# micahvista/VACmap

Measured on AMD Instinct MI355X. Metric: aligned Gbp/s (whole node) + reads/s, 15 kb ONT-shape reads vs hg38-size ref, 1/2/4/8 MI355X, higher is better.
Workload: dtype i16/i32 DP + f64 chains

## Files before the change

### include/vacmapx.h

```cpp
#ifndef VACMAPX_H
#define VACMAPX_H
#include <stdint.h>
#ifdef __cplusplus
extern "C" {
#endif

typedef enum vm_status {
    VM_OK = 0,
    VM_ERR_ARG = -1,
    VM_ERR_NO_DEVICE = -2,
    VM_ERR_NO_CTX = -3,
    VM_ERR_OOM = -4,
    VM_ERR_IO = -5,
    VM_ERR_HIP = -6,
    VM_ERR_UNSUPPORTED = -7,
    VM_READ_RAISED = -10,
    VM_READ_CAPACITY = -20,
    VM_READ_FASTPATH = -21,
    VM_READ_UNSUPPORTED = -22
} vm_status;

enum { VM_MODE_H = 0, VM_MODE_L = 1, VM_MODE_S = 2, VM_MODE_R = 3,
       VM_MODE_ASM = 4 };

// ... 65 lines not shown
    double* S; int64_t* P; int64_t* S_arg; int64_t* gmax; int64_t* opcount;
} vm_chains_out;
int vm_chain_global_batch(vm_ctx*, const vm_params*, int kmersize, int64_t n, const int64_t* anchors,
                          const int64_t* anchor_off, const int64_t* readlens, int want_raw, vm_chains_out* out);
void vm_chains_out_free(vm_chains_out*);

typedef struct vm_local_out {
    int32_t* status;
    int32_t* variant;
    double* score;
    int64_t* chain_off;
    int64_t* chain;
    int64_t* raw_off;
    int64_t* raw;
} vm_local_out;
int vm_local_chain_batch(vm_ctx*, const vm_index*, const vm_params*, int64_t n, const char* seqs, const int64_t* offsets,
                         const int64_t* read_path_off, const int64_t* path_off, const int64_t* path_anchors, vm_local_out* out);
void vm_local_out_free(vm_local_out*);

typedef struct vm_linked_out {
    int64_t gmax, n_hot, n_cold, opcount; double cold_max;
    double* S; int64_t* P; int64_t* S_arg_hot;
    int32_t carry_status, saved; int64_t n_carry; double* carry_S; int64_t* carry_P; int64_t* carry_rows; double carry_g_max_scores; int64_t carry_prereadloc;
} vm_linked_out;
int vm_chain_linked(vm_ctx*, int which, int kmersize, double skipcost, int maxdiff, int maxgap, int64_t n, const int64_t* rows, int64_t n_pre,
                    const double* pre_S, const int64_t* pre_P, double g_max_scores, int64_t g_max_index, int64_t prereadloc, vm_linked_out* out);
void vm_linked_out_free(vm_linked_out*);

typedef struct vm_score { int32_t match, mismatch, o1, e1, o2, e2; } vm_score;
int vm_k_cigar_batch(vm_ctx*, const vm_score*, int eqx, int64_t n, const char* t, const int64_t* t_off, const char* q,
                     const int64_t* q_off, char** cigars, int64_t** cigar_off, int32_t** scores);
int vm_k_cigar_batch_banded(vm_ctx*, const vm_score*, int eqx, int64_t n, const char* t, const int64_t* t_off, const char* q,
                            const int64_t* q_off, char** cigars, int64_t** cigar_off, int32_t** band_flag, int64_t* stats);
int vm_k_extend_batch(vm_ctx*, int match, int mismatch, int o, int e, int bw, int zdrop, int64_t n, const char* t,
                      const int64_t* t_off, const char* q, const int64_t* q_off, int32_t** t_e, int32_t** q_e, int32_t** score);
typedef struct vm_cigar_out { char* cigar; int32_t q_e, t_e, score; } vm_cigar_out;
int vm_k_cigar(vm_ctx*, const char* t, int64_t tl, const char* q, int64_t ql, const vm_score* sc, int bw, int zdrop,
               int eqx, vm_cigar_out* out);
int vm_edit_distance_batch(vm_ctx*, int64_t n, const char* q, const int64_t* q_off, const char* t, const int64_t* t_off,
                           int64_t** dist);
int64_t vm_edit_distance(vm_ctx*, const char* q, int64_t ql, const char* t, int64_t tl);
int vm_edit_distance_bound_batch(vm_ctx*, int tier, int64_t n, const char* q, const int64_t* q_off, const char* t, const int64_t* t_off,
                                 int64_t** bound);

typedef struct vm_record {
    int32_t read_idx;
    int32_t contig;
    int32_t strand;
    int32_t mapq;
    int64_t q_st, q_en;
    int64_t r_st, r_en;
    int64_t cigar_off, cigar_len;
} vm_record;

typedef struct vm_batch_stats {
    int64_t n_reads, read_bases, n_minimizers, n_hits, n_anchors, n_local_hits, n_local_anchors;
    int64_t n_segments, n_ed_problems, ed_cells, n_ext_problems, ext_cells, n_dp_problems, dp_cells;
    int64_t n_records, cigar_bytes, aligned_bases, n_unmapped, n_failed;
    int64_t dp_string_bytes;
    double ms_total;
    double ms_stage[16];
    double ms_gapfill_fill;
    double ms_gapfill_trace;
    int64_t n_gapfill_launches;
    int64_t n_ed_full;
    int64_t n_ed_tier2;
// ... 76 lines not shown
```

### vacmap_amd/csrc/k_dp.hip

```cpp
#include "vmx_device.h"
#include "vmx_kernels.h"

__device__ __forceinline__ int vmx_tcode(uint8_t c) { return c < 4 ? (int)c : 6; }


__global__ void k_encode(const char* __restrict__ in, uint8_t* __restrict__ out, int64_t n) {
    int64_t i = (int64_t)blockIdx.x * blockDim.x + threadIdx.x;
    int64_t stride = (int64_t)gridDim.x * blockDim.x;
    for (; i < n; i += stride) out[i] = vmx_code((uint8_t)in[i]);
}

#define VMX_EXT_RING 512
__global__ void __launch_bounds__(64) k_extend(const uint8_t* __restrict__ tcodes, const int64_t* __restrict__ t_off,
                                               const uint8_t* __restrict__ qcodes, const int64_t* __restrict__ q_off, int n_prob,
                                               int match, int mismatch, int o, int e, int bw_in, int zdrop,
                                               int32_t* __restrict__ out_te, int32_t* __restrict__ out_qe, int32_t* __restrict__ out_sc, const int32_t* __restrict__ n_ptr) {
    if (n_ptr) n_prob = *n_ptr;
    __shared__ int sH[3][VMX_EXT_RING];
    __shared__ int sE[2][VMX_EXT_RING];
    __shared__ int sF[2][VMX_EXT_RING];
    const int lane = vmx_lane();
    const int RM = VMX_EXT_RING - 1;
    for (int p = blockIdx.x; p < n_prob; p += gridDim.x) {
        const uint8_t* T = tcodes + t_off[p];
// ... 239 lines not shown
                    sHE = (unsigned)vmx_r16_ror1((int)vmx_bfi(l15, (outH >> 16) | (outE1 & 0xffff0000u), sHE));                    \
                    sE2 = (unsigned)vmx_r16_ror1((int)vmx_bfi(l15, outE2 >> 16, sE2));                                             \
                    if ((TT) == 14) {       \
                        const int colr = t + 14 - 30 - l;           \
                        const int col = colr;                                                                                      \
                        if (store_bnd && act && colr >= 1 && col <= ql) { bH[col] = (int)(short)(sHE & 0xffffu); bE1[col] = (int)sHE >> 16; bE2[col] = (int)(short)(sE2 & 0xffffu); } \
                    }                                                                                                              \
                }                                                                                                                  \
            }
        const int tfin_rel = act ? t_fin - t : -1;
        if (__any(act && t < 32)) {
            VMX_X4_STEP(true, 0) VMX_X4_STEP(true, 1) VMX_X4_STEP(true, 2) VMX_X4_STEP(true, 3) VMX_X4_STEP(true, 4) VMX_X4_STEP(true, 5) VMX_X4_STEP(true, 6) VMX_X4_STEP(true, 7)
            VMX_X4_STEP(true, 8) VMX_X4_STEP(true, 9) VMX_X4_STEP(true, 10) VMX_X4_STEP(true, 11) VMX_X4_STEP(true, 12) VMX_X4_STEP(true, 13) VMX_X4_STEP(true, 14) VMX_X4_STEP(true, 15)
        } else {
            VMX_X4_STEP(false, 0) VMX_X4_STEP(false, 1) VMX_X4_STEP(false, 2) VMX_X4_STEP(false, 3) VMX_X4_STEP(false, 4) VMX_X4_STEP(false, 5) VMX_X4_STEP(false, 6) VMX_X4_STEP(false, 7)
            VMX_X4_STEP(false, 8) VMX_X4_STEP(false, 9) VMX_X4_STEP(false, 10) VMX_X4_STEP(false, 11) VMX_X4_STEP(false, 12) VMX_X4_STEP(false, 13) VMX_X4_STEP(false, 14) VMX_X4_STEP(false, 15)
        }
#undef VMX_X4_STEP
        if (act) {
            t += 16; tbp += 16 * 32;
            if (t == W) {
                const int colr = W - 31 - l, col = colr;
                if (store_bnd && colr > ((W - 31) & ~15) && col <= ql) { bH[col] = (int)(short)(sHE & 0xffffu); bE1[col] = (int)sHE >> 16; bE2[col] = (int)(short)(sE2 & 0xffffu); }
                t = 0; ++s;
            }
        }
    }
    const int sc = (rf & 1) ? vmx_pk_hi(fin) : vmx_pk_lo(fin);
    if (SCORE && nstr > 0 && l == (rf >> 1)) *score_out = sc;
    return sc;
}

#include "vmx_dp_ad.h"

template <bool SCORE>
__device__ __forceinline__ void vmx_gapfill_fill_one(const uint8_t* __restrict__ tcodes, const uint8_t* __restrict__ qcodes, const vmx_dp_prob* __restrict__ probs, int p,
                                                    int match, int mismatch, int o1, int e1, int o2, int e2, uint8_t* __restrict__ tb_pool,
                                                    int32_t* __restrict__ bnd_pool, int32_t* __restrict__ out_score, int lane, int flag_value = 0, uint8_t* __restrict__ redo_pool = nullptr) {
        const vmx_dp_prob pr = probs[p];
        const uint8_t* T = tcodes + pr.t_off;
        const uint8_t* Q = qcodes + pr.q_off;
        const int tl = vmx_uniform_i32(pr.tl), ql = vmx_uniform_i32(pr.ql);
        const bool trivial = tl == 0 || ql == 0;
        if (trivial && lane == 0) out_score[p] = (tl + ql) ? vmx_gap_open_row(tl + ql, o1, e1, o2, e2) : 0;
        if (!SCORE && !trivial && lane == 0) out_score[p] = flag_value;
        uint8_t* tb = vmx_tb_ptr(tb_pool, redo_pool, pr.tb_off);
        int32_t* bH = bnd_pool + pr.bnd_off;
        int32_t* bE1 = bH + (ql + 1);
        int32_t* bE2 = bE1 + (ql + 1);
        const bool pk = !trivial && VMX_DP16_OK(tl, ql);
        const int W = ql + 63;
        const int nstr = (trivial || pk) ? 0 : (tl + 63) >> 6;
        int outH = 0;
        for (int s = 0; s < nstr; ++s) {
            const int i = s * 64 + lane + 1;
            const int ti = i <= tl ? (int)T[i - 1] : 4;
            int Hleft = vmx_gap_open_row(i, o1, e1, o2, e2);
            int F1 = VMX_NEG, F2 = VMX_NEG;
            int Hdiag = (i - 1 == 0) ? 0 : vmx_gap_open_row(i - 1, o1, e1, o2, e2);
            int outE1 = VMX_NEG, outE2 = VMX_NEG;
            outH = 0;
            int qc_cur = 4;
            int sH = 0, sE1 = 0, sE2 = 0;
            const bool store_bnd = s + 1 < nstr;
            uint8_t* tbs = tb + (size_t)s * (size_t)W * 64 + lane;
#define VMX_GF_STEP(PRED)                                                                                             \
// ... 20 lines not shown
                    tbs[(size_t)t * 64] = (uint8_t)(b | src);                                                         \
                    Hdiag = upH; Hleft = h;                                                                           \
                    outH = h; outE1 = e1v; outE2 = e2v;                                                               \
                }                                                                                                     \
                if (store_bnd) {                                                                                      \
                    sH = vmx_ror1(lane == 63 ? outH : sH); sE1 = vmx_ror1(lane == 63 ? outE1 : sE1); sE2 = vmx_ror1(lane == 63 ? outE2 : sE2); \
                    const int j63 = t - 62;                                         \
                    if (j63 >= 1 && j63 <= ql && ((j63 & 63) == 0 || j63 == ql)) {                                    \
                        const int col = j63 - lane;                      \
                        if (col > ((j63 - 1) & ~63)) { bH[col] = sH; bE1[col] = sE1; bE2[col] = sE2; }                \
                    }                                                                                                 \
                }                                                                                                     \
            }
            for (int t0 = 0; t0 < W; t0 += 64) {
                const int jj = t0 + lane;
                int qchunk = jj < ql ? (int)Q[jj] : 4;
                int cH = 0, cE1 = VMX_NEG, cE2 = VMX_NEG;
                if (jj + 1 <= ql) {
                    if (s == 0) cH = vmx_gap_open_row(jj + 1, o1, e1, o2, e2);
                    else { cH = bH[jj + 1]; cE1 = bE1[jj + 1]; cE2 = bE2[jj + 1]; }
                }
                if (t0 >= 64 && t0 + 64 <= ql) {
                    for (int tt = 0; tt < 64; ++tt) { const int t = t0 + tt; VMX_GF_STEP(true) }
                } else {
                    int tend = W - t0; if (tend > 64) tend = 64;
                    for (int tt = 0; tt < tend; ++tt) { const int t = t0 + tt; const int j = t - lane + 1; VMX_GF_STEP(j >= 1 && j <= ql) }
                }
            }
#undef VMX_GF_STEP
            __syncthreads();
        }
        if (!trivial && !pk && lane == ((tl - 1) & 63)) out_score[p] = outH;
        int32_t sink = 0;
        if (pk) vmx_gapfill_fill16(T, Q, tl, ql, match, mismatch, o1, e1, o2, e2, tb, bH, SCORE ? &out_score[p] : &sink, lane);
}

template <bool SCORE>
__device__ __forceinline__ void vmx_gapfill_fill_body(const uint8_t* __restrict__ tcodes, const uint8_t* __restrict__ qcodes,
                                                     const vmx_dp_prob* __restrict__ probs, int n_prob, int match, int mismatch,
                                                     int o1, int e1, int o2, int e2, uint8_t* __restrict__ tb_pool,
                                                     int32_t* __restrict__ bnd_pool, int32_t* __restrict__ out_score,
                                                     const int32_t* __restrict__ order, int32_t* __restrict__ counter,
                                                     int32_t* __restrict__ redo_list = nullptr, int32_t* __restrict__ redo_cnt = nullptr, int redo_pass = 0,
                                                     uint8_t* __restrict__ redo_pool = nullptr) {
    const int lane = vmx_lane();
    int static_next = 4 * (int)blockIdx.x;
    if (redo_pass) {
        n_prob = redo_cnt[0]; order = redo_list; counter = redo_cnt + 1;
        while (true) {
            int q; { int v = 0; if (lane == 0) v = atomicAdd(redo_cnt + 2, 1); q = vmx_bcast0(v); }
            if (q >= n_prob) break;
            const int p = order[q];
            const int tl = probs[p].tl, ql = probs[p].ql;
            if (VMX_REDO_PK(tl, ql)) vmx_gapfill_fill_one<SCORE>(tcodes, qcodes, probs, p, match, mismatch, o1, e1, o2, e2, tb_pool, bnd_pool, out_score, lane, VMX_PK_FLAG, redo_pool);
        }
    }
    while (true) {
        int q0;
        if (order) { int v = 0; if (lane == 0) v = atomicAdd(counter, 4); q0 = vmx_bcast0(v); }
        else { q0 = static_next; static_next += 4 * (int)gridDim.x; }
        if (q0 >= n_prob) break;
        const int qg = q0 + (lane >> 4);
        const int pg = qg < n_prob ? (order ? order[qg] : qg) : -1;
        bool x4 = false, skip = false;
        {
            vmx_dp_prob pr; pr.tl = 0; pr.ql = 0; pr.t_off = 0; pr.q_off = 0; pr.tb_off = 0; pr.bnd_off = 0;
            if (pg >= 0) pr = probs[pg];
// ... 61 lines not shown
            if (x4X) {
                out_score[pX] = keepX ? VMX_AD_FLAG + ns : 0;
                if (!keepX) {
                    if (triedX) atomicAdd(redo_cnt + 3, 1);
                    const unsigned long long need = (unsigned long long)VMX_REDO_TB_BYTES(prX.tl, prX.ql), at = atomicAdd(redo_bytes, need);
                    if (at + need > redo_cap) { probs[pX].tl = 0; probs[pX].ql = 0; probs[pX].tb_off = 0; }
                    else { probs[pX].tb_off = -(int64_t)at - 1; redo_list[atomicAdd(redo_cnt, 1)] = pX; }
                }
            }
            if (x4Y) {
                out_score[pY] = keepY ? VMX_AD_FLAG + ns : 0;
                if (!keepY) {
                    if (triedY) atomicAdd(redo_cnt + 3, 1);
                    const unsigned long long need = (unsigned long long)VMX_REDO_TB_BYTES(prY.tl, prY.ql), at = atomicAdd(redo_bytes, need);
                    if (at + need > redo_cap) { probs[pY].tl = 0; probs[pY].ql = 0; probs[pY].tb_off = 0; }
                    else { probs[pY].tb_off = -(int64_t)at - 1; redo_list[atomicAdd(redo_cnt, 1)] = pY; }
                }
            }
        }
        for (int gk = 0; gk < 8; ++gk) {
            const int p = vmx_readlane((gk & 1) ? pY : pX, 16 * (gk >> 1));
            if (p < 0 || vmx_readlane((int)((gk & 1) ? x4Y : x4X), 16 * (gk >> 1))) continue;
            vmx_gapfill_fill_one<false>(tcodes, qcodes, probs, p, match, mismatch, o1, e1, o2, e2, tb_pool, bnd_pool, out_score, lane);
        }
    }
}

__global__ void __launch_bounds__(64) k_gapfill_fill(const uint8_t* __restrict__ tcodes, const uint8_t* __restrict__ qcodes,
                                                     const vmx_dp_prob* __restrict__ probs, int n_prob, int match, int mismatch,
                                                     int o1, int e1, int o2, int e2, uint8_t* __restrict__ tb_pool,
                                                     int32_t* __restrict__ bnd_pool, int32_t* __restrict__ out_score,
                                                     const int32_t* __restrict__ order, int32_t* __restrict__ counter) {
    vmx_gapfill_fill_body<true>(tcodes, qcodes, probs, n_prob, match, mismatch, o1, e1, o2, e2, tb_pool, bnd_pool, out_score, order, counter);
}
__global__ void __launch_bounds__(64, 4) k_gapfill_fill_ns(const uint8_t* __restrict__ tcodes, const uint8_t* __restrict__ qcodes,
                                                        vmx_dp_prob* __restrict__ probs, int n_prob, int match, int mismatch,
                                                        int o1, int e1, int o2, int e2, uint8_t* __restrict__ tb_pool,
                                                        int32_t* __restrict__ bnd_pool, int32_t* __restrict__ out_score,
                                                        const int32_t* __restrict__ order, const int32_t* __restrict__ range, int32_t* __restrict__ counter,
                                                        int32_t* __restrict__ redo_list, int32_t* __restrict__ redo_cnt, int redo_pass, int ad_pct,
                                                        uint8_t* __restrict__ redo_pool, unsigned long long* __restrict__ redo_bytes, const int32_t* __restrict__ n_ptr,
                                                        unsigned long long redo_cap, int tb_by_ns) {
    if (n_ptr) n_prob = *n_ptr;
    if (redo_pass) vmx_gapfill_fill_body<false>(tcodes, qcodes, probs, n_prob, match, mismatch, o1, e1, o2, e2, tb_pool, bnd_pool, out_score, order, counter, redo_list, redo_cnt, 1, redo_pool);
    else vmx_gapfill_ad_pass(tcodes, qcodes, probs, n_prob, match, mismatch, o1, e1, o2, e2, tb_pool, bnd_pool, out_score, order, range, counter, redo_list, redo_cnt, ad_pct, redo_bytes, redo_cap, tb_by_ns);
}

__global__ void k_gapfill_trace(const uint8_t* __restrict__ tcodes, const uint8_t* __restrict__ qcodes,
                                const vmx_dp_prob* __restrict__ probs, int n_prob, int eqx, const uint8_t* __restrict__ tb_pool,
                                uint32_t* __restrict__ run_pool, char* __restrict__ cig_pool, int32_t* __restrict__ cig_len,
                                const int32_t* __restrict__ band_flag, const uint8_t* __restrict__ redo_pool, int spread, int32_t* __restrict__ cig_q,
                                const int32_t* __restrict__ n_ptr) {
    VMX_SETPRIO(3);
    if (n_ptr) n_prob = *n_ptr;
    const int gt = (int)(blockIdx.x * blockDim.x + threadIdx.x);
    if (spread > 1 && gt % spread) return;
    int p = spread > 1 ? gt / spread : gt;
    if (p >= n_prob) return;
    const vmx_dp_prob pr = probs[p];
    const uint8_t* T = tcodes + pr.t_off;
    const uint8_t* Q = qcodes + pr.q_off;
    const int tl = pr.tl, ql = pr.ql;
    const uint8_t* tb = vmx_tb_ptr(tb_pool, redo_pool, pr.tb_off);
    uint32_t* runs = run_pool + pr.run_off;
    char* cig = cig_pool + pr.cig_off;
    bool x4 = tl > 0 && ql > 0 && VMX_DP16X4_OK(tl, ql);
// ... 75 lines not shown
```

### vacmap_amd/csrc/vmx_capi.hip

```cpp
#include "vmx_host.h"
#include <time.h>
#include "vmx_select.h"
#include "vmx_stage.h"
#include "vmx_round.h"
#include <algorithm>
#include <cmath>
#include <cstdlib>
#include <cstring>
#include <numeric>

namespace vmx {
static thread_local std::string g_err;
void set_error(const std::string& s) { g_err = s; }
int hip_fail(hipError_t e, const char* what, const char* file, int line) {
    g_err = std::string("HIP error: ") + hipGetErrorString(e) + " at " + what + " (" + file + ":" + std::to_string(line) + ")";
    return e == hipErrorOutOfMemory ? VM_ERR_OOM : VM_ERR_HIP;
}
}
using namespace vmx;

void vmx_ctx_free_local_bufs(vm_ctx* c);
void vmx_ctx_free_batch_bufs(vm_ctx* c);

static inline int grid_for(const vm_ctx* c, int64_t n_items, int per_cu = 8) {
// ... 452 lines not shown
    VMX_TRY(upload_encode(c, q, q_off, n, c->b[3], c->b[4], c->b[5]));
    std::vector<vmx_dp_prob> probs((size_t)n);
    int64_t tb = 0, bnd = 0, run = 0, cig = 0;
    for (int64_t i = 0; i < n; ++i) {
        vmx_dp_prob& p = probs[i];
        p.t_off = t_off[i]; p.q_off = q_off[i]; p.tl = (int32_t)(t_off[i + 1] - t_off[i]); p.ql = (int32_t)(q_off[i + 1] - q_off[i]);
        p.tb_off = tb; p.bnd_off = bnd; p.run_off = run; p.cig_off = cig;
        tb += VMX_TB_BYTES((int64_t)p.tl, (int64_t)p.ql);
        bnd += 3 * (int64_t)(p.ql + 1); run += (int64_t)p.tl + p.ql + 2; cig += 2 * ((int64_t)p.tl + p.ql) + 16;
    }
    VMX_TRY(upload(c->b[6], probs.data(), (size_t)n, c->stream));
    VMX_TRY(c->b[7].reserve((size_t)tb + 64)); VMX_TRY(c->b[8].reserve(sizeof(int32_t) * (size_t)(bnd + 4)));
    VMX_TRY(c->b[9].reserve(sizeof(uint32_t) * (size_t)(run + 4))); VMX_TRY(c->b[10].reserve((size_t)cig + 16));
    VMX_TRY(c->b[11].reserve(sizeof(int32_t) * 2 * (size_t)(n + 1)));
    int32_t* d_score = c->b[11].as<int32_t>(); int32_t* d_len = d_score + n;
    if (n) {
        hipLaunchKernelGGL(k_gapfill_fill, dim3(grid_for(c, n, 16)), dim3(64), 0, c->stream, c->b[1].as<uint8_t>(), c->b[4].as<uint8_t>(),
                           c->b[6].as<vmx_dp_prob>(), (int)n, sc->match, sc->mismatch, sc->o1, sc->e1, sc->o2, sc->e2, c->b[7].as<uint8_t>(),
                           c->b[8].as<int32_t>(), d_score, (const int32_t*)nullptr, (int32_t*)nullptr);
        hipLaunchKernelGGL(k_gapfill_trace, dim3((unsigned)((n + 63) / 64)), dim3(64), 0, c->stream, c->b[1].as<uint8_t>(), c->b[4].as<uint8_t>(),
                           c->b[6].as<vmx_dp_prob>(), (int)n, eqx, c->b[7].as<uint8_t>(), c->b[9].as<uint32_t>(), c->b[10].as<char>(), d_len, (const int32_t*)nullptr, (const uint8_t*)nullptr, 1, (int32_t*)nullptr);
    }
    std::vector<char> hc((size_t)cig + 16); std::vector<int32_t> hl((size_t)n);
    *scores = host_alloc<int32_t>((size_t)n);
    VMX_TRY(download(hc.data(), c->b[10].p, (size_t)cig, c->stream));
    VMX_TRY(download(hl.data(), d_len, (size_t)n, c->stream));
    VMX_TRY(download(*scores, d_score, (size_t)n, c->stream));
    VMX_HIP(hipStreamSynchronize(c->stream));
    VMX_HIP(hipGetLastError());
    cigar_strings(n, probs.data(), hc.data(), hl.data(), cigars, cigar_off);
    return VM_OK;
}

int vm_k_cigar_batch_banded(vm_ctx* c, const vm_score* sc, int eqx, int64_t n, const char* t, const int64_t* t_off, const char* q,
                            const int64_t* q_off, char** cigars, int64_t** cigar_off, int32_t** band_flag, int64_t* stats) {
    if (!c) { set_error("no context"); return VM_ERR_NO_CTX; }
    if (n > 0x7fffffff) { set_error("too many problems"); return VM_ERR_ARG; }
    VMX_HIP(hipSetDevice(c->device));
    vmx_fetch_scope fetch_scope(c);
    vmx_batch_bufs& B = *vmx_ctx_batch_bufs(c);
    VMX_TRY(upload_encode(c, t, t_off, n, c->b[0], B.tpool, c->b[2]));
    VMX_TRY(upload_encode(c, q, q_off, n, c->b[3], B.qpool, c->b[5]));
    const int ad_pct = vmx_ad_pct_env();
    vmx_round_args R; memset(&R, 0, sizeof R);
    R.ad_on = 1; R.ad_match = sc->match; R.ad_o1 = sc->o1; R.ad_e1 = sc->e1; R.ad_o2 = sc->o2; R.ad_e2 = sc->e2; R.ad_pct = ad_pct;
    std::vector<vmx_dp_prob> probs((size_t)n);
    std::vector<int64_t> keys((size_t)n);
    int64_t tb = 0, bnd = 0, run = 0, cig = 0, redo = 0;
    for (int64_t i = 0; i < n; ++i) {
        vmx_dp_prob& p = probs[i];
        p.t_off = t_off[i]; p.q_off = q_off[i]; p.tl = (int32_t)(t_off[i + 1] - t_off[i]); p.ql = (int32_t)(q_off[i + 1] - q_off[i]);
        p.tb_off = tb; p.bnd_off = bnd; p.run_off = run; p.cig_off = cig;
        tb += vmx_round_tb_bytes(R, p.tl, p.ql); keys[i] = vmx_round_key(R, p.tl, p.ql);
        if (p.tl > 0 && p.ql > 0 && VMX_DP16X4_OK(p.tl, p.ql)) redo += VMX_REDO_TB_BYTES((int64_t)p.tl, (int64_t)p.ql);
        bnd += 3 * (int64_t)(p.ql + 1); run += (int64_t)p.tl + p.ql + 2; cig += 2 * ((int64_t)p.tl + p.ql) + 16;
    }
    const int32_t nn = (int32_t)n;
    VMX_TRY(upload(B.dptab, probs.data(), (size_t)n, c->stream)); VMX_TRY(upload(B.dpsz[0], keys.data(), (size_t)n, c->stream)); VMX_TRY(upload(B.chunkn, &nn, 1, c->stream));
    VMX_TRY(B.tb.reserve((size_t)tb + 64)); VMX_TRY(B.tbredo.reserve((size_t)redo + 64)); VMX_TRY(B.bnd.reserve(sizeof(int32_t) * (size_t)(bnd + 4)));
    VMX_TRY(B.run.reserve(sizeof(uint32_t) * (size_t)(run + 4))); VMX_TRY(B.cig.reserve((size_t)cig + 16));
    VMX_TRY(B.ciglen.reserve(4 * (size_t)(n + 1))); VMX_TRY(B.cigq.reserve(4 * (size_t)(n + 1))); VMX_TRY(B.dpscore.reserve(4 * (size_t)(n + 1)));
    VMX_TRY(B.order.reserve(4 * (size_t)(2 * n + 64)));
    VMX_TRY(B.gfctl.reserve(4 * VMX_GF_SLOT)); VMX_HIP(hipMemsetAsync(B.gfctl.p, 0, 4 * VMX_GF_SLOT, c->stream));
    if (n) vmx_gapfill_chunk(c, B, *sc, ad_pct, eqx, 0, n, B.chunkn.as<int32_t>(), 0, B.gfctl.as<int32_t>(), B.order.as<int32_t>() + n + 32, redo, nullptr);
    std::vector<char> hc((size_t)cig + 16); std::vector<int32_t> hl((size_t)n), flag((size_t)n), ctl(32);
    VMX_TRY(download(hc.data(), B.cig.p, (size_t)cig, c->stream));
// ... 109 lines not shown
```

### vacmap_amd/csrc/vmx_dp_ad.h

```cpp
#ifndef VMX_DP_AD_H
#define VMX_DP_AD_H

#ifdef VMX_EMU
__device__ __forceinline__ int vmx_r16_shl1_in(int v, int in) { const int l = vmx_lane(); const int e = __shfl(v, (l & 48) | ((l + 1) & 15)); return (l & 15) == 15 ? in : e; }
__device__ __forceinline__ unsigned vmx_perm(unsigned s0, unsigned s1, unsigned sel) {
    unsigned r = 0;
    for (int b = 0; b < 4; ++b) {
        const unsigned c = (sel >> (8 * b)) & 0xffu;
        const unsigned v = c < 4 ? (s1 >> (8 * c)) & 0xffu : c < 8 ? (s0 >> (8 * (c - 4))) & 0xffu : 0u;
        r |= v << (8 * b);
    }
    return r;
}
#else
__device__ __forceinline__ int vmx_r16_shl1_in(int v, int in) { return __builtin_amdgcn_update_dpp(in, v, 0x101, 0xf, 0xf, false); }
__device__ __forceinline__ unsigned vmx_perm(unsigned s0, unsigned s1, unsigned sel) { return __builtin_amdgcn_perm(s0, s1, sel); }
#endif

#define VMX_AD_NEGINF (-4096)
#define VMX_AD_CSH 12
#define VMX_AD_TE1 6u
#define VMX_AD_TF1 3u
#define VMX_AD_TE2 1u
#define VMX_AD_TF2 0u
__host__ __device__ constexpr long long vmx_ad_imax(long long a, long long b) { return a > b ? a : b; }
__host__ __device__ constexpr long long vmx_ad_imin(long long a, long long b) { return a < b ? a : b; }
__host__ __device__ constexpr long long vmx_ad_bias(int mismatch, int o1, int e1, int o2, int e2) {
    return -((long long)VMX_AD_NEGINF - (long long)(VMX_DP16X4_MAX + 1) * vmx_ad_imax(e1, e2) - vmx_ad_imax(vmx_ad_imax(o1, o2), -(long long)mismatch));
}
__host__ __device__ constexpr bool vmx_ad_scores_ok(int match, int mismatch, int o1, int e1, int o2, int e2) {
    return match >= 0 && mismatch <= match && 8LL * (match - mismatch) <= (1 << VMX_AD_CSH) && o1 >= 0 && e1 >= 0 && o2 >= 0 && e2 >= 0 &&
           (long long)match * (VMX_DP16X4_MAX / 2 + 1) + vmx_ad_bias(mismatch, o1, e1, o2, e2) <= 8191 &&
           vmx_ad_imin(mismatch, 0) * (VMX_DP16X4_MAX / 2) - vmx_ad_imin(o1 + (long long)e1 * VMX_DP16X4_MAX, o2 + (long long)e2 * VMX_DP16X4_MAX)
               - vmx_ad_imax(o1, o2) - vmx_ad_imax(e1, e2) > (long long)VMX_AD_NEGINF + vmx_ad_imax(o1, o2);
}
static_assert(vmx_ad_scores_ok(2, -4, 4, 2, 24, 1), "the gap fill's own scoring (vmx_align.hip: gf_score) must fit the tagged 16-bit domain");
struct vmx_ad_consts { unsigned O1, O2, E1, E2, MATCH, PEN, NH, NE1, NE2, NF1, NF2; };

__device__ __forceinline__ void vmx_ad_cell(const vmx_ad_consts& K, unsigned upH, unsigned upE1, unsigned upE2, unsigned leftH, unsigned leftF1,
                                            unsigned leftF2, unsigned tc, unsigned qc, unsigned& H, unsigned& E1, unsigned& E2, unsigned& F1, unsigned& F2,
                                            unsigned (&w)[5]) {
    const unsigned e1v = vmx_pk_max_u16(upH - K.O1, upE1) - K.E1, e2v = vmx_pk_max_u16(upH - K.O2, upE2) - K.E2;
    const unsigned f1v = vmx_pk_max_u16(leftH - K.O1, leftF1) - K.E1, f2v = vmx_pk_max_u16(leftH - K.O2, leftF2) - K.E2;
    E1 = e1v & ~((7u ^ VMX_AD_TE1) * 0x00010001u); E2 = e2v & ~((7u ^ VMX_AD_TE2) * 0x00010001u);
    F1 = f1v & ~((7u ^ VMX_AD_TF1) * 0x00010001u); F2 = f2v & ~((7u ^ VMX_AD_TF2) * 0x00010001u);
    const unsigned hd = H + K.MATCH - vmx_pk_min_u16(tc ^ qc, K.PEN);
    const unsigned h = vmx_pk_max_u16(vmx_pk_max_u16(hd, E1), vmx_pk_max_u16(vmx_pk_max_u16(F1, E2), F2));
    H = h | 0x00070007u;
    w[0] = h; w[1] = e1v; w[2] = e2v; w[3] = f1v; w[4] = f2v;
}

__device__ __forceinline__ unsigned vmx_ad_bytes(const unsigned (&a)[5], const unsigned (&b)[5]) {
    constexpr unsigned SEL = 0x06020400u;
    const unsigned gh = vmx_perm(b[0], a[0], SEL), ge1 = vmx_perm(b[1], a[1], SEL), ge2 = vmx_perm(b[2], a[2], SEL);
    const unsigned gf1 = vmx_perm(b[3], a[3], SEL), gf2 = vmx_perm(b[4], a[4], SEL);
    const unsigned src = vmx_perm(0x00010000u, 0x03000204u, gh & 0x07070707u);
    unsigned op = vmx_bfi(0x01010101u, ge1, ge2);
    op = vmx_bfi(0x04040404u, gf1, op);
    op = vmx_bfi(0x08080808u, (gf2 << 3) | (gf2 >> 29), op);
    return src | (((op & 0x0f0f0f0fu) ^ 0x0f0f0f0fu) << 3);
}

template <int NS>
__device__ __forceinline__ void vmx_ad_pack(const unsigned (&w)[NS][5], unsigned& w01, unsigned& w23) {
    w01 = vmx_ad_bytes(w[0], w[NS > 1 ? 1 : 0]);
    w23 = 0;
    if (NS > 2) w23 = vmx_ad_bytes(w[NS > 2 ? 2 : 0], w[NS > 3 ? 3 : 0]);
    if (NS == 3) w23 &= 0x00ff00ffu;
}

// ... 135 lines not shown
```

### vacmap_amd/csrc/vmx_host.h

```cpp
#ifndef VMX_HOST_H
#define VMX_HOST_H
#include "vmx_device.h"
#include "vmx_kernels.h"
#include "../../include/vacmapx.h"
#include <algorithm>
#include <map>
#include <cstring>
#include <string>
#include <vector>
#include <chrono>
#include <atomic>
#include <mutex>
#include <execinfo.h>

namespace vmx {

void set_error(const std::string& s);
int hip_fail(hipError_t e, const char* what, const char* file, int line);

#define VMX_HIP(expr)                                                              \
    do {                                                                           \
        hipError_t _e = (expr);                                                    \
        if (_e != hipSuccess) return vmx::hip_fail(_e, #expr, __FILE__, __LINE__);  \
    } while (0)
// ... 210 lines not shown
        for (int i = 0; i < n; ++i) { (void)hipEventRecord(c->join_ev[i], c->aux[i]); (void)hipStreamWaitEvent(c->stream, c->join_ev[i], 0); }
        used = 0;
    }
};

__global__ void k_encode(const char* in, uint8_t* out, int64_t n);
__global__ void k_edit_distance(const uint8_t* qcodes, const int64_t* q_off, const uint8_t* tcodes, const int64_t* t_off,
                                int8_t* carry_pool, const int32_t* order, const int32_t* range, int32_t* counters, int which, int64_t* out,
                                int64_t carry_stride, int32_t* oflow);
__global__ void k_size_order(const int64_t* size, const int32_t* n_ptr, int64_t thresh, int32_t* order, int32_t* range, int32_t* counters);
__global__ void k_size_hist(const int64_t* size, const int32_t* n_ptr, int64_t thresh, int32_t* ghist);
__global__ void k_size_scatter(const int64_t* size, const int32_t* n_ptr, const int32_t* ghist, int32_t* gcur, int32_t* order, int32_t* range, int32_t* counters);
static inline void vmx_size_order_wide(vm_ctx* c, const int64_t* size, const int32_t* n_ptr, int64_t n_upper, int64_t thresh, int32_t* order, int32_t* range, int32_t* counters,
                                       int32_t* scratch) {
    static const bool one_wg = getenv("VMX_SIZE_ORDER_ONE") != nullptr;
    if (one_wg) { hipLaunchKernelGGL(k_size_order, dim3(1), dim3(1024), 0, c->stream, size, n_ptr, thresh, order, range, counters); return; }
    (void)hipMemsetAsync(scratch, 0, 4 * 513, c->stream);
    const unsigned G = (unsigned)std::max<int64_t>(1, std::min<int64_t>((n_upper + 1023) / 1024, (int64_t)c->num_cu * 2));
    hipLaunchKernelGGL(k_size_hist, dim3(G), dim3(256), 0, c->stream, size, n_ptr, thresh, scratch);
    hipLaunchKernelGGL(k_size_scatter, dim3(G), dim3(256), 0, c->stream, size, n_ptr, (const int32_t*)scratch, scratch + 257, order, range, counters);
}
__global__ void k_ed_banded(const uint8_t* qcodes, const int64_t* q_off, const uint8_t* tcodes, const int64_t* t_off, const int32_t* order,
                            const int32_t* range, int32_t* counter, int64_t* ub_out);
struct vmx_ext_args;
__global__ void k_ed_banded4(const uint8_t* qcodes, const int64_t* q_off, const uint8_t* tcodes, const int64_t* t_off, const int32_t* order,
                             const int32_t* range, int32_t* counter, int64_t* ub_out);
__global__ void k_ed_flag(const int64_t* ub, const int64_t* q_off, const int64_t* t_off, const int32_t* n_ptr, double maxdiv, int64_t* sizes,
                          int64_t* ed_out, int32_t* n_flagged, int first, const int32_t* prob_read, struct vmx_ext_read* er);
__global__ void k_extend(const uint8_t* tcodes, const int64_t* t_off, const uint8_t* qcodes, const int64_t* q_off, int n_prob,
                         int match, int mismatch, int o, int e, int bw_in, int zdrop, int32_t* out_te, int32_t* out_qe, int32_t* out_sc, const int32_t* n_ptr);
__global__ void k_gapfill_fill(const uint8_t* tcodes, const uint8_t* qcodes, const vmx_dp_prob* probs, int n_prob, int match,
                               int mismatch, int o1, int e1, int o2, int e2, uint8_t* tb_pool, int32_t* bnd_pool, int32_t* out_score,
                               const int32_t* order, int32_t* counter);
__global__ void k_gapfill_fill_ns(const uint8_t* tcodes, const uint8_t* qcodes, vmx_dp_prob* probs, int n_prob, int match,
                                  int mismatch, int o1, int e1, int o2, int e2, uint8_t* tb_pool, int32_t* bnd_pool, int32_t* out_score,
                                  const int32_t* order, const int32_t* range, int32_t* counter, int32_t* redo_list, int32_t* redo_cnt, int redo_pass, int ad_pct,
                                  uint8_t* redo_pool, unsigned long long* redo_bytes, const int32_t* n_ptr = nullptr, unsigned long long redo_cap = ~0ULL, int tb_by_ns = 0);
static inline int vmx_ad_pct_env(int mode = 0) {
    int pct = mode == 1 ? 40 : 90, pmin = mode == 1 ? 40 : VMX_AD_PCT_MIN_DEFAULT;
    if (const char* e = getenv("VMX_AD_PCT")) { const int v = atoi(e); if (v >= 0 && v <= 60000) pct = v; }
    if (const char* e = getenv("VMX_AD_PCT_MIN")) { const int v = atoi(e); if (v >= 0 && v <= 60000) pmin = v; }
    return pct | (pmin << 16);
}
__global__ void k_gapfill_trace(const uint8_t* tcodes, const uint8_t* qcodes, const vmx_dp_prob* probs, int n_prob, int eqx,
                                const uint8_t* tb_pool, uint32_t* run_pool, char* cig_pool, int32_t* cig_len, const int32_t* band_flag, const uint8_t* redo_pool, int spread, int32_t* cig_q, const int32_t* n_ptr = nullptr);
__global__ void k_flip_sort(const int64_t* rows, const int64_t* aoff, const int64_t* readlens, int n_reads, uint64_t* key_pool,
                            const int64_t* key_off, vmx_anchor* sorted, int32_t* need_reverse);
__global__ void k_chain_global(const vmx_anchor* anchors, const int64_t* aoff, const int32_t* rlist, int nlist, int lds_cap,
                               vmx_tables tab, const double* gapcost_list, double oskipcost, int omaxdiff, int maxgap,
                               double* S_out, int32_t* P_out, int32_t* SA_out, uint8_t* cov_pool, int64_t* gmax_out, int64_t* opcount_out, int rmode,
                               double* FP_pool, double* PP_pool);
__global__ void k_chain_global_rows(const vmx_anchor* anchors, const int64_t* aoff, const int32_t* rlist, int nlist, vmx_tables tab, const double* gapcost_list,
                                    double oskipcost, int omaxdiff, int maxgap, double* S_out, int32_t* P_out, int32_t* SA_out, uint8_t* cov_pool,
                                    int64_t* gmax_out, int64_t* opcount_out, int rmode, double* FP_pool, double* PP_pool, unsigned long long* dbg);
__global__ void k_chain_global_rows_w3(const vmx_anchor* anchors, const int64_t* aoff, const int32_t* rlist, int nlist, vmx_tables tab, const double* gapcost_list,
                                       double oskipcost, int omaxdiff, int maxgap, double* S_out, int32_t* P_out, int32_t* SA_out, uint8_t* cov_pool,
                                       int64_t* gmax_out, int64_t* opcount_out, int rmode, double* FP_pool, double* PP_pool, unsigned long long* dbg);
static inline bool vmx_chain_rows_win3() { const char* e = getenv("VMX_RW_WIN"); return e && atoi(e) == 3; }
unsigned long long* vmx_chain_dbg();
void vmx_chain_dbg_report(hipStream_t st);
static inline bool vmx_chain_rows_on() { static const bool on = [] { const char* e = getenv("VMX_CHAIN_ROWS"); return !e || atoi(e) != 0; }(); return on; }
__global__ void k_chain_global_fast(const vmx_anchor* anchors, const int64_t* aoff, int n_reads, const int64_t* roff, vmx_tables tab,
                                    const double* gapcost_list, double oskipcost, int omaxdiff, int maxgap, double* S_out, int32_t* P_out, int32_t* SA_out,
                                    uint8_t* cov_pool, int32_t* si_pool, int64_t* t_pool, int32_t* cnt_pool, int64_t* gmax_out, int32_t* ran, int rmode,
                                    double* FP_pool, double* PP_pool);
__global__ void k_chain_select(const vmx_anchor* anchors, const int64_t* aoff, const int64_t* readlens, const int32_t* rlist, int nlist, int lds_cap,
// ... 6 lines not shown
```

### vacmap_amd/lib.py

```python
import ctypes as C
import os
import numpy as np

_HERE = os.path.dirname(os.path.abspath(__file__))
DEFAULT_SO = os.environ.get('VACMAPX_LIB') or os.path.join(_HERE, 'libvacmapx.so')

VM_ERR_NO_DEVICE = -2
MODES = {'H': 0, 'L': 1, 'S': 2, 'R': 3, 'asm': 4}


class VmxError(RuntimeError):
    def __init__(self, code, msg):
        super().__init__('vacmapx error %d: %s' % (code, msg))
        self.code = code


class Params(C.Structure):
    _fields_ = [('mode', C.c_int32), ('check_num', C.c_int32), ('mid_occ', C.c_int32), ('global_maxdiff', C.c_int32),
                ('local_maxdiff', C.c_int32), ('local_kmersize', C.c_int32), ('eqx', C.c_int32), ('hardclip', C.c_int32),
                ('nodiscard', C.c_int32), ('reserved', C.c_int32), ('global_skipcost', C.c_double),
                ('local_skipcost', C.c_double), ('maxdivergence', C.c_double)]


class Score(C.Structure):
# ... 253 lines not shown
        t, to = _cat(targets); q, qo = _cat(queries)
        te = C.POINTER(C.c_int32)(); qe = C.POINTER(C.c_int32)(); sc = C.POINTER(C.c_int32)()
        n = len(targets)
        self.lib.check(self.lib.L.vm_k_extend_batch(self.h, match, mismatch, o, e, bw, zdrop, n, t, to.ctypes.data, q, qo.ctypes.data,
                                                    C.byref(te), C.byref(qe), C.byref(sc)))
        return self._take(sc, n, np.int32), self._take(te, n, np.int32), self._take(qe, n, np.int32)

    def k_cigar_batch(self, targets, queries, match=2, mismatch=-4, o1=4, e1=2, o2=24, e2=1, eqx=False):
        t, to = _cat(targets); q, qo = _cat(queries)
        n = len(targets)
        sc = Score(match, mismatch, o1, e1, o2, e2)
        cg = C.c_void_p(); co = C.POINTER(C.c_int64)(); ss = C.POINTER(C.c_int32)()
        self.lib.check(self.lib.L.vm_k_cigar_batch(self.h, C.byref(sc), int(eqx), n, t, to.ctypes.data, q, qo.ctypes.data,
                                                   C.byref(cg), C.byref(co), C.byref(ss)))
        off = self._take(co, n + 1, np.int64)
        blob = C.string_at(cg.value, int(off[-1])) if off[-1] else b''
        self.lib.L.vm_free(cg)
        cigars = [blob[off[i]:off[i + 1] - 1].decode() for i in range(n)]
        return cigars, self._take(ss, n, np.int32)

    def k_cigar_batch_banded(self, targets, queries, match=2, mismatch=-4, o1=4, e1=2, o2=24, e2=1, eqx=False):
        t, to = _cat(targets); q, qo = _cat(queries)
        n = len(targets)
        sc = Score(match, mismatch, o1, e1, o2, e2)
        cg = C.c_void_p(); co = C.POINTER(C.c_int64)(); fl = C.POINTER(C.c_int32)(); st = (C.c_int64 * 4)()
        self.lib.check(self.lib.L.vm_k_cigar_batch_banded(self.h, C.byref(sc), int(eqx), n, t, to.ctypes.data, q, qo.ctypes.data,
                                                          C.byref(cg), C.byref(co), C.byref(fl), st))
        off = self._take(co, n + 1, np.int64)
        blob = C.string_at(cg.value, int(off[-1])) if off[-1] else b''
        self.lib.L.vm_free(cg)
        cigars = [blob[off[i]:off[i + 1] - 1].decode() for i in range(n)]
        return cigars, self._take(fl, n, np.int32), {'eligible': st[0], 'proven': st[1], 'redo': st[2], 'not_eligible': st[3]}

    def k_cigar(self, target, query, match=2, mismatch=-4, gap_open_1=4, gap_extend_1=2, gap_open_2=24, gap_extend_2=1,
                bw=-1, zdropvalue=-1, eqx=False):
        t, q = _b(target), _b(query)
        sc = Score(match, mismatch, gap_open_1, gap_extend_1, gap_open_2, gap_extend_2)
        out = CigarOut()
        self.lib.check(self.lib.L.vm_k_cigar(self.h, t, len(t), q, len(q), C.byref(sc), bw, zdropvalue, int(eqx), C.byref(out)))
        cg = C.string_at(out.cigar).decode() if out.cigar else ''
        self.lib.L.vm_free(out.cigar)
        return cg, 0, out.q_e, out.t_e, 0, 0

    def chain_global_batch(self, prm, kmersize, anchors_list, readlens, want_raw=False):
        n = len(anchors_list)
        aoff = np.zeros(n + 1, np.int64)
        for i, a in enumerate(anchors_list):
            aoff[i + 1] = aoff[i] + len(a)
        rows = np.ascontiguousarray(np.concatenate([np.asarray(a, dtype=np.int64).reshape(-1, 4) for a in anchors_list]) if n else np.zeros((0, 4), np.int64))
        rl = np.ascontiguousarray(readlens, dtype=np.int64)
        out = ChainsOut()
        self.lib.check(self.lib.L.vm_chain_global_batch(self.h, C.byref(prm), kmersize, n, rows.ctypes.data, aoff.ctypes.data, rl.ctypes.data,
                                                        int(want_raw), C.byref(out)))
        res = []
        rpo = np.ctypeslib.as_array(out.read_path_off, shape=(n + 1,)).copy()
        npaths = int(rpo[-1])
        po = np.ctypeslib.as_array(out.path_off, shape=(npaths + 1,)).copy()
        nrows = int(po[-1])
        pa = np.ctypeslib.as_array(out.path_anchors, shape=(max(nrows, 1), 4))[:nrows].copy()
        tot = int(aoff[-1])
        for r in range(n):
            d = {'need_reverse': bool(out.need_reverse[r]), 'mapq': int(out.mapq[r]), 'score': float(out.score[r]),
                 'fast_used': bool(out.fast_used[r]), 'gmax': int(out.gmax[r]), 'opcount': int(out.opcount[r]),
                 'paths': [pa[po[p]:po[p + 1]] for p in range(rpo[r], rpo[r + 1])]}
            if want_raw:
                a, b = int(aoff[r]), int(aoff[r + 1])
# ... 563 lines not shown
```

Measured before the change: 3.465.

## Add tagged 16-bit packed gap-fill DP that encodes traceback in score low bits

Adds a tagged full-matrix fill in which each 16-bit score carries a 3-bit origin tag in its low bits (scores scaled by 8 plus a bias), so max selection also yields the traceback direction. It uses a 128-row strip (two rows per lane) instead of the previous packed form, and it is used whenever the problem's score range fits the tagged domain. The aim is fewer instructions per cell for traceback generation and fewer strips. In exchange it narrows the usable score range and adds a debug C API that fills a single problem.

```diff
diff --git a/include/vacmapx.h b/include/vacmapx.h
--- a/include/vacmapx.h
+++ b/include/vacmapx.h
@@ -121,6 +121,8 @@
                      const int64_t* q_off, char** cigars, int64_t** cigar_off, int32_t** scores);
 int vm_k_cigar_batch_banded(vm_ctx*, const vm_score*, int eqx, int64_t n, const char* t, const int64_t* t_off, const char* q,
                             const int64_t* q_off, char** cigars, int64_t** cigar_off, int32_t** band_flag, int64_t* stats);
+int vm_k_fill16_tb(vm_ctx*, const vm_score*, int tagged, const char* t, int64_t tl, const char* q, int64_t ql, uint8_t** tb, int64_t* tb_bytes,
+                   int32_t* score);
 int vm_k_extend_batch(vm_ctx*, int match, int mismatch, int o, int e, int bw, int zdrop, int64_t n, const char* t,
                       const int64_t* t_off, const char* q, const int64_t* q_off, int32_t** t_e, int32_t** q_e, int32_t** score);
 typedef struct vm_cigar_out { char* cigar; int32_t q_e, t_e, score; } vm_cigar_out;
diff --git a/vacmap_amd/csrc/k_dp.hip b/vacmap_amd/csrc/k_dp.hip
--- a/vacmap_amd/csrc/k_dp.hip
+++ b/vacmap_amd/csrc/k_dp.hip
@@ -295,6 +295,82 @@
 }
 
 #include "vmx_dp_ad.h"
+
+
+__device__ __forceinline__ unsigned vmx_pkt_bytes(const unsigned (&w)[5]) {
+    const unsigned src = vmx_perm(0x00010000u, 0x03000204u, w[0] & 0x00070007u);
+    unsigned op = vmx_bfi(0x00010001u, w[1], w[2]);
+    op = vmx_bfi(0x00040004u, w[3], op);
+    op = vmx_bfi(0x00080008u, w[4] << 3, op);
+    return vmx_pk_bytes(src | (((op & 0x000f000fu) ^ 0x000f000fu) << 3));
+}
+__device__ __forceinline__ void vmx_gapfill_fill16_tag(const uint8_t* __restrict__ T, const uint8_t* __restrict__ Q, int tl, int ql, int match, int mismatch,
+                                                       int o1, int e1, int o2, int e2, uint8_t* __restrict__ tb, int32_t* __restrict__ bH,
+                                                       int32_t* __restrict__ score_out, int lane) {
+    int32_t* bE1 = bH + (ql + 1);
+    int32_t* bE2 = bE1 + (ql + 1);
+    const int W = ql + 127;
+    const int nstr = (tl + 127) >> 7;
+    vmx_ad_consts K;
+    K.O1 = vmx_pk(8 * o1, 8 * o1); K.O2 = vmx_pk(8 * o2, 8 * o2); K.E1 = vmx_pk(8 * e1, 8 * e1); K.E2 = vmx_pk(8 * e2, 8 * e2);
+    K.MATCH = vmx_pk(8 * match, 8 * match); K.PEN = vmx_pk(8 * (match - mismatch), 8 * (match - mismatch));
+    const int bias = (int)vmx_pkt_bias(tl + ql, mismatch, o1, e1, o2, e2);
+    auto tg = [&](int v, unsigned tag) -> unsigned { return 8u * (unsigned)(v + bias) + tag; };
+    const unsigned NE1 = VMX_AD_TE1 * 0x00010001u, NE2 = VMX_AD_TE2 * 0x00010001u, NF1 = VMX_AD_TF1 * 0x00010001u, NF2 = VMX_AD_TF2 * 0x00010001u;
+    const unsigned ZERO = tg(0, 7u) * 0x00010001u;
+    const int rf = (tl - 1) & 127;
+    const int t_fin = ql - 1 + rf;
+    unsigned fin = 0;
+    for (int s = 0; s < nstr; ++s) {
+        const int i0 = s * 128 + 2 * lane + 1;
+        const unsigned ti2 = vmx_pk((i0 <= tl ? vmx_tcode(T[i0 - 1]) : 5) << VMX_AD_CSH, (i0 + 1 <= tl ? vmx_tcode(T[i0]) : 5) << VMX_AD_CSH);
+        unsigned Hleft = tg(vmx_gap_open_row(i0, o1, e1, o2, e2), 7u) | (tg(vmx_gap_open_row(i0 + 1, o1, e1, o2, e2), 7u) << 16);
+        unsigned F1 = NF1, F2 = NF2;
+        unsigned Hdiag = tg(i0 - 1 == 0 ? 0 : vmx_gap_open_row(i0 - 1, o1, e1, o2, e2), 7u) | (tg(vmx_gap_open_row(i0, o1, e1, o2, e2), 7u) << 16);
+        unsigned outH = ZERO, outE1 = NE1, outE2 = NE2, qc = vmx_pk(4 << VMX_AD_CSH, 4 << VMX_AD_CSH);
+        int sH = 0, sE1 = 0, sE2 = 0;
+        const bool store_bnd = s + 1 < nstr;
+        uint8_t* tbs = tb + (size_t)s * (size_t)W * 128 + 2 * lane;
+        for (int t0 = 0; t0 < W; t0 += 64) {
+            const int jj = t0 + lane;
+            unsigned qchunk = (unsigned)((jj < ql ? (int)Q[jj] : 4) << VMX_AD_CSH) << 16;
+            unsigned cH = ZERO << 16, cE1 = NE1 << 16, cE2 = NE2 << 16;
+            if (jj + 1 <= ql) {
+                if (s == 0) cH = tg(vmx_gap_open_row(jj + 1, o1, e1, o2, e2), 7u) << 16;
+                else { cH = tg(bH[jj + 1], 7u) << 16; cE1 = tg(bE1[jj + 1], VMX_AD_TE1) << 16; cE2 = tg(bE2[jj + 1], VMX_AD_TE2) << 16; }
+            }
+            int tend = W - t0; if (tend > 64) tend = 64;
+            const bool ramp_up = t0 < 128;
+            for (int tt = 0; tt < tend; ++tt) {
+                const int t = t0 + tt;
+                const unsigned upH = vmx_alignbit16(outH, (unsigned)vmx_shr1_in((int)outH, (int)cH));
+                const unsigned upE1 = vmx_alignbit16(outE1, (unsigned)vmx_shr1_in((int)outE1, (int)cE1));
+                const unsigned upE2 = vmx_alignbit16(outE2, (unsigned)vmx_shr1_in((int)outE2, (int)cE2));
+                qc = vmx_alignbit16(qc, (unsigned)vmx_shr1_in((int)qc, (int)qchunk));
+                cH = (unsigned)vmx_rol1((int)cH); cE1 = (unsigned)vmx_rol1((int)cE1); cE2 = (unsigned)vmx_rol1((int)cE2); qchunk = (unsigned)vmx_rol1((int)qchunk);
+                unsigned h = Hdiag, nE1, nE2, nF1, nF2, w[5];
+                vmx_ad_cell(K, upH, upE1, upE2, Hleft, F1, F2, ti2, qc, h, nE1, nE2, nF1, nF2, w);
+                *(uint16_t*)(tbs + (size_t)t * 128) = (uint16_t)vmx_pkt_bytes(w);
+                if (ramp_up) {
+                    const unsigned pm = (t >= 2 * lane ? 0xffffu : 0u) | (t >= 2 * lane + 1 ? 0xffff0000u : 0u);
+                    Hdiag = vmx_bfi(pm, upH, Hdiag); Hleft = vmx_bfi(pm, h, Hleft); F1 = vmx_bfi(pm, nF1, F1); F2 = vmx_bfi(pm, nF2, F2);
+                } else { Hdiag = upH; Hleft = h; F1 = nF1; F2 = nF2; }
+                outH = h; outE1 = nE1; outE2 = nE2;
+                fin = (t == t_fin) ? outH : fin;
+                if (store_bnd) {
+                    sH = vmx_ror1(lane == 63 ? (int)(outH >> 16) : sH); sE1 = vmx_ror1(lane == 63 ? (int)(outE1 >> 16) : sE1); sE2 = vmx_ror1(lane == 63 ? (int)(outE2 >> 16) : sE2);
+                    const int j63 = t - 126;
+                    if (j63 >= 1 && j63 <= ql && ((j63 & 63) == 0 || j63 == ql)) {
+                        const int col = j63 - lane;
+                        if (col > ((j63 - 1) & ~63)) { bH[col] = (sH >> 3) - bias; bE1[col] = (sE1 >> 3) - bias; bE2[col] = (sE2 >> 3) - bias; }
+                    }
+                }
+            }
+        }
+        __syncthreads();
+    }
+    if (lane == (rf >> 1)) *score_out = (int)(((rf & 1) ? fin >> 16 : fin & 0xffffu) >> 3) - bias;
+}
 
 template <bool SCORE>
 __device__ __forceinline__ void vmx_gapfill_fill_one(const uint8_t* __restrict__ tcodes, const uint8_t* __restrict__ qcodes, const vmx_dp_prob* __restrict__ probs, int p,
@@ -381,7 +457,8 @@
         }
         if (!trivial && !pk && lane == ((tl - 1) & 63)) out_score[p] = outH;
         int32_t sink = 0;
-        if (pk) vmx_gapfill_fill16(T, Q, tl, ql, match, mismatch, o1, e1, o2, e2, tb, bH, SCORE ? &out_score[p] : &sink, lane);
+        if (pk && vmx_pkt_ok(tl + ql, match, mismatch, o1, e1, o2, e2)) vmx_gapfill_fill16_tag(T, Q, tl, ql, match, mismatch, o1, e1, o2, e2, tb, bH, SCORE ? &out_score[p] : &sink, lane);
+        else if (pk) vmx_gapfill_fill16(T, Q, tl, ql, match, mismatch, o1, e1, o2, e2, tb, bH, SCORE ? &out_score[p] : &sink, lane);
 }
 
 template <bool SCORE>
@@ -509,6 +586,14 @@
                                                      int32_t* __restrict__ bnd_pool, int32_t* __restrict__ out_score,
                                                      const int32_t* __restrict__ order, int32_t* __restrict__ counter) {
     vmx_gapfill_fill_body<true>(tcodes, qcodes, probs, n_prob, match, mismatch, o1, e1, o2, e2, tb_pool, bnd_pool, out_score, order, counter);
+}
+__global__ void __launch_bounds__(64) k_gapfill_fill16_one(const uint8_t* __restrict__ T, const uint8_t* __restrict__ Q, int tl, int ql, int match, int mismatch,
+                                                           int o1, int e1, int o2, int e2, uint8_t* __restrict__ tb, int32_t* __restrict__ bnd,
+                                                           int32_t* __restrict__ out_score, int tagged) {
+    const int lane = vmx_lane();
+    if (tagged && !vmx_pkt_ok(tl + ql, match, mismatch, o1, e1, o2, e2)) { if (lane == 0) *out_score = INT32_MIN; return; }
+    if (tagged) vmx_gapfill_fill16_tag(T, Q, tl, ql, match, mismatch, o1, e1, o2, e2, tb, bnd, out_score, lane);
+    else vmx_gapfill_fill16(T, Q, tl, ql, match, mismatch, o1, e1, o2, e2, tb, bnd, out_score, lane);
 }
 __global__ void __launch_bounds__(64, 4) k_gapfill_fill_ns(const uint8_t* __restrict__ tcodes, const uint8_t* __restrict__ qcodes,
                                                         vmx_dp_prob* __restrict__ probs, int n_prob, int match, int mismatch,
diff --git a/vacmap_amd/csrc/vmx_capi.hip b/vacmap_amd/csrc/vmx_capi.hip
--- a/vacmap_amd/csrc/vmx_capi.hip
+++ b/vacmap_amd/csrc/vmx_capi.hip
@@ -508,6 +508,27 @@
     return VM_OK;
 }
 
+int vm_k_fill16_tb(vm_ctx* c, const vm_score* sc, int tagged, const char* t, int64_t tl, const char* q, int64_t ql, uint8_t** tb, int64_t* tb_bytes, int32_t* score) {
+    if (!c) { set_error("no context"); return VM_ERR_NO_CTX; }
+    if (tl < 1 || ql < 1 || !VMX_DP16_OK(tl, ql)) { set_error("vm_k_fill16_tb: the packed form takes 1 <= tl, ql and tl + ql <= VMX_DP16_MAX"); return VM_ERR_ARG; }
+    VMX_HIP(hipSetDevice(c->device));
+    const int64_t to[2] = {0, tl}, qo[2] = {0, ql};
+    VMX_TRY(upload_encode(c, t, to, 1, c->b[0], c->b[1], c->b[2]));
+    VMX_TRY(upload_encode(c, q, qo, 1, c->b[3], c->b[4], c->b[5]));
+    const int64_t nb = VMX_PK_TB_BYTES(tl, ql);
+    VMX_TRY(c->b[7].reserve((size_t)nb + 64)); VMX_TRY(c->b[8].reserve(sizeof(int32_t) * (size_t)(3 * (ql + 1) + 4))); VMX_TRY(c->b[11].reserve(sizeof(int32_t) * 4));
+    VMX_HIP(hipMemsetAsync(c->b[7].p, 0xff, (size_t)nb, c->stream));
+    hipLaunchKernelGGL(k_gapfill_fill16_one, dim3(1), dim3(64), 0, c->stream, c->b[1].as<uint8_t>(), c->b[4].as<uint8_t>(), (int)tl, (int)ql, sc->match, sc->mismatch,
+                       sc->o1, sc->e1, sc->o2, sc->e2, c->b[7].as<uint8_t>(), c->b[8].as<int32_t>(), c->b[11].as<int32_t>(), tagged);
+    *tb = host_alloc<uint8_t>((size_t)nb + 1); *tb_bytes = nb;
+    VMX_TRY(download(*tb, c->b[7].p, (size_t)nb, c->stream));
+    VMX_TRY(download(score, c->b[11].p, 1, c->stream));
+    VMX_HIP(hipStreamSynchronize(c->stream));
+    VMX_HIP(hipGetLastError());
+    if (*score == INT32_MIN) { free(*tb); *tb = nullptr; set_error("vm_k_fill16_tb: the scores of this problem do not fit the tagged domain (vmx_pkt_ok)"); return VM_ERR_UNSUPPORTED; }
+    return VM_OK;
+}
+
 int vm_k_cigar_batch_banded(vm_ctx* c, const vm_score* sc, int eqx, int64_t n, const char* t, const int64_t* t_off, const char* q,
                             const int64_t* q_off, char** cigars, int64_t** cigar_off, int32_t** band_flag, int64_t* stats) {
     if (!c) { set_error("no context"); return VM_ERR_NO_CTX; }
diff --git a/vacmap_amd/csrc/vmx_dp_ad.h b/vacmap_amd/csrc/vmx_dp_ad.h
--- a/vacmap_amd/csrc/vmx_dp_ad.h
+++ b/vacmap_amd/csrc/vmx_dp_ad.h
@@ -36,6 +36,17 @@
 }
 static_assert(vmx_ad_scores_ok(2, -4, 4, 2, 24, 1), "the gap fill's own scoring (vmx_align.hip: gf_score) must fit the tagged 16-bit domain");
 struct vmx_ad_consts { unsigned O1, O2, E1, E2, MATCH, PEN, NH, NE1, NE2, NF1, NF2; };
+
+__host__ __device__ constexpr long long vmx_pkt_bias(int per, int mismatch, int o1, int e1, int o2, int e2) {
+    return vmx_ad_imin(2LL * o1 + ((long long)per + 256) * e1, 2LL * o2 + ((long long)per + 256) * e2) +
+           vmx_ad_imax(vmx_ad_imax(o1, o2) + vmx_ad_imax(e1, e2), -(long long)mismatch) + 1;
+}
+__host__ __device__ constexpr bool vmx_pkt_ok(int per, int match, int mismatch, int o1, int e1, int o2, int e2) {
+    return match >= 0 && mismatch <= 0 && 8LL * (match - mismatch) <= (1 << VMX_AD_CSH) && o1 >= 0 && e1 >= 0 && o2 >= 0 && e2 >= 0 &&
+           (long long)match * (per / 2 + 1) + vmx_pkt_bias(per, mismatch, o1, e1, o2, e2) <= 8191;
+}
+static_assert(vmx_pkt_ok(VMX_DP16X4_MAX, 2, -4, 4, 2, 24, 1), "every problem the second launch fills on a whole wave (VMX_REDO_PK) must fit the tagged domain");
+static_assert(vmx_pkt_ok(3929, 2, -4, 4, 2, 24, 1) && !vmx_pkt_ok(3930, 2, -4, 4, 2, 24, 1), "the tagged full-matrix form's range under the gap fill's scoring");
 
 __device__ __forceinline__ void vmx_ad_cell(const vmx_ad_consts& K, unsigned upH, unsigned upE1, unsigned upE2, unsigned leftH, unsigned leftF1,
                                             unsigned leftF2, unsigned tc, unsigned qc, unsigned& H, unsigned& E1, unsigned& E2, unsigned& F1, unsigned& F2,
diff --git a/vacmap_amd/csrc/vmx_host.h b/vacmap_amd/csrc/vmx_host.h
--- a/vacmap_amd/csrc/vmx_host.h
+++ b/vacmap_amd/csrc/vmx_host.h
@@ -266,6 +266,8 @@
 __global__ void k_gapfill_fill(const uint8_t* tcodes, const uint8_t* qcodes, const vmx_dp_prob* probs, int n_prob, int match,
                                int mismatch, int o1, int e1, int o2, int e2, uint8_t* tb_pool, int32_t* bnd_pool, int32_t* out_score,
                                const int32_t* order, int32_t* counter);
+__global__ void k_gapfill_fill16_one(const uint8_t* T, const uint8_t* Q, int tl, int ql, int match, int mismatch, int o1, int e1, int o2, int e2, uint8_t* tb,
+                                     int32_t* bnd, int32_t* out_score, int tagged);
 __global__ void k_gapfill_fill_ns(const uint8_t* tcodes, const uint8_t* qcodes, vmx_dp_prob* probs, int n_prob, int match,
                                   int mismatch, int o1, int e1, int o2, int e2, uint8_t* tb_pool, int32_t* bnd_pool, int32_t* out_score,
                                   const int32_t* order, const int32_t* range, int32_t* counter, int32_t* redo_list, int32_t* redo_cnt, int redo_pass, int ad_pct,
diff --git a/vacmap_amd/lib.py b/vacmap_amd/lib.py
--- a/vacmap_amd/lib.py
+++ b/vacmap_amd/lib.py
@@ -309,6 +309,17 @@
         cigars = [blob[off[i]:off[i + 1] - 1].decode() for i in range(n)]
         return cigars, self._take(fl, n, np.int32), {'eligible': st[0], 'proven': st[1], 'redo': st[2], 'not_eligible': st[3]}
 
+    def k_fill16_tb(self, target, query, match=2, mismatch=-4, o1=4, e1=2, o2=24, e2=1, tagged=True):
+        t, q = _b(target), _b(query)
+        sc = Score(match, mismatch, o1, e1, o2, e2)
+        f = self.lib.L.vm_k_fill16_tb
+        f.argtypes = [C.c_void_p, C.POINTER(Score), C.c_int, C.c_char_p, C.c_int64, C.c_char_p, C.c_int64, C.POINTER(C.c_void_p), C.POINTER(C.c_int64), C.POINTER(C.c_int32)]
+        tb = C.c_void_p(); nb = C.c_int64(); s = C.c_int32()
+        self.lib.check(f(self.h, C.byref(sc), int(tagged), t, len(t), q, len(q), C.byref(tb), C.byref(nb), C.byref(s)))
+        raw = C.string_at(tb.value, nb.value)
+        self.lib.L.vm_free(tb)
+        return np.frombuffer(raw, dtype=np.uint8), s.value
+
     def k_cigar(self, target, query, match=2, mismatch=-4, gap_open_1=4, gap_extend_1=2, gap_open_2=24, gap_extend_2=1,
                 bw=-1, zdropvalue=-1, eqx=False):
         t, q = _b(target), _b(query)
```

After: 3.388. 0.978x the previous value.
